# avlmaps/AVLMaps

Measured on AMD Instinct MI355X. Metric: voxel_query_similarities_per_sec, higher is better.
Workload: dtype f32

## Files before the change

avlmaps_amd/csrc/avl_sim.hip:

```cpp
#include <cfloat>
#include <algorithm>
#include <climits>
#include <cstdlib>
#include <vector>

#include "avl_common.h"

namespace avl {

using half8 = __attribute__((ext_vector_type(8))) _Float16;
using half2 = __attribute__((ext_vector_type(2))) _Float16;
using f32x16 = __attribute__((ext_vector_type(16))) float;
using f32x4 = __attribute__((ext_vector_type(4))) float;

constexpr int kExactQB = 8;

template <bool VEC4>
__global__ __launch_bounds__(256) void sim_exact_kernel(const float* __restrict__ feat, int64_t N, int D, int64_t ld,
                                                        const float* __restrict__ q, int Q, int64_t ldq, int q0,
                                                        float* __restrict__ scores, int32_t* __restrict__ argmax,
                                                        float* __restrict__ best, int first_chunk) {
    extern __shared__ __attribute__((aligned(16))) float qs[];
    const int Dp = (D + 3) & ~3;
    const int qn = min(kExactQB, Q - q0);
    for (int i = threadIdx.x; i < kExactQB * Dp; i += blockDim.x) {
        int j = i / Dp, d = i - j * Dp;
        qs[i] = (j < qn && d < D) ? q[(int64_t)(q0 + j) * ldq + d] : 0.f;
    }
    __syncthreads();

    const int lane = threadIdx.x & 63;
    const int64_t wave = (int64_t)blockIdx.x * (blockDim.x >> 6) + (threadIdx.x >> 6);
    const int64_t nwaves = (int64_t)gridDim.x * (blockDim.x >> 6);
    constexpr int R = 4;

    for (int64_t row0 = wave * R; row0 < N; row0 += nwaves * R) {
// ... 148 lines not shown
    const float x[8] = {v0.x, v0.y, v0.z, v0.w, v1.x, v1.y, v1.z, v1.w};
    float m1 = -1.0f;
    asm("" : "+v"(m1));
#pragma unroll
    for (int p = 0; p < 4; ++p) {
        half2 h = __builtin_bit_cast(half2, __builtin_amdgcn_cvt_pkrtz(x[2 * p], x[2 * p + 1]));
        float r0 = __builtin_fmaf((float)h[0], m1, x[2 * p]);
        float r1 = __builtin_fmaf((float)h[1], m1, x[2 * p + 1]);
        half2 l = __builtin_bit_cast(half2, __builtin_amdgcn_cvt_pkrtz(r0, r1));
        hi[2 * p] = h[0];
        hi[2 * p + 1] = h[1];
        lo[2 * p] = l[0];
        lo[2 * p + 1] = l[1];
    }
#endif
}

constexpr float kGuardLo = 0x1p-7f, kGuardHi = 0x1p15f;

__device__ __forceinline__ void guard_max8(float& m, const f32x4 v0, const f32x4 v1) {
#ifndef AVL_GUARD_BUILTIN
    asm("v_max3_f32 %0, |%1|, |%2|, %0" : "+v"(m) : "v"(v0.x), "v"(v0.y));
    asm("v_max3_f32 %0, |%1|, |%2|, %0" : "+v"(m) : "v"(v0.z), "v"(v0.w));
    asm("v_max3_f32 %0, |%1|, |%2|, %0" : "+v"(m) : "v"(v1.x), "v"(v1.y));
    asm("v_max3_f32 %0, |%1|, |%2|, %0" : "+v"(m) : "v"(v1.z), "v"(v1.w));
#else
    m = __builtin_fmaxf(__builtin_fmaxf(m, __builtin_fabsf(v0.x)), __builtin_fabsf(v0.y));
    m = __builtin_fmaxf(__builtin_fmaxf(m, __builtin_fabsf(v0.z)), __builtin_fabsf(v0.w));
    m = __builtin_fmaxf(__builtin_fmaxf(m, __builtin_fabsf(v1.x)), __builtin_fabsf(v1.y));
    m = __builtin_fmaxf(__builtin_fmaxf(m, __builtin_fabsf(v1.z)), __builtin_fabsf(v1.w));
#endif
}

template <int QT, int NA, bool XR = false>
__device__ __forceinline__ void split_epilogue(const f32x16 (&acc)[QT][NA], const float* isc, int q_base, int rows, int Q,
                                               float* __restrict__ scores, int32_t* __restrict__ argmax,
                                               float* __restrict__ best, int64_t row, int64_t N, int kg, int first_chunk,
                                               float rscale = 1.f, uint32_t* __restrict__ flags = nullptr, float rmax = 1.f,
                                               const int32_t* qml = nullptr, f32x4 xacc = f32x4{0.f, 0.f, 0.f, 0.f}) {
    int lim = (XR ? 32 * QT : rows) - 4 * kg;
    asm volatile("" : "+v"(lim));
    float bv = -INFINITY;
    int bl = INT_MAX;
#pragma unroll
    for (int t = 0; t < QT; ++t) {
#pragma unroll
        for (int g = 0; g < 4; ++g) {
            const int c0 = t * 32 + 8 * g;
            const int ql = c0 + 4 * kg;
            const int qg = q_base + ql;
            const f32x4 is4 = *reinterpret_cast<const f32x4*>(isc + ql);
            f32x4 v;
            f32x4 r = {acc[t][0][4 * g + 0], acc[t][0][4 * g + 1], acc[t][0][4 * g + 2], acc[t][0][4 * g + 3]};
#pragma unroll
            for (int a = 1; a < NA; ++a) {
                r.x += acc[t][a][4 * g + 0]; r.y += acc[t][a][4 * g + 1]; r.z += acc[t][a][4 * g + 2]; r.w += acc[t][a][4 * g + 3];
            }
            v.x = r.x * is4.x * rscale;
            v.y = r.y * is4.y * rscale;
            v.z = r.z * is4.z * rscale;
            v.w = r.w * is4.w * rscale;
            if (scores && row < N) {
                float* sp = scores + row * (int64_t)Q + qg;
                if (qml) {
                    float* sr = scores + row * (int64_t)Q;
                    const int4 qm4 = *reinterpret_cast<const int4*>(qml + ql);
                    if (c0 + 0 < lim) sr[qm4.x] = v.x;
                    if (c0 + 1 < lim) sr[qm4.y] = v.y;
                    if (c0 + 2 < lim) sr[qm4.z] = v.z;
                    if (c0 + 3 < lim) sr[qm4.w] = v.w;
                } else if (c0 + 3 < lim && (Q & 3) == 0) {
                    *reinterpret_cast<f32x4*>(sp) = v;
                } else {
                    if (c0 + 0 < lim) sp[0] = v.x;
                    if (c0 + 1 < lim) sp[1] = v.y;
                    if (c0 + 2 < lim) sp[2] = v.z;
                    if (c0 + 3 < lim) sp[3] = v.w;
                }
            }
            if (c0 + 0 < lim && v.x > bv) { bv = v.x; bl = c0 + 0; }
            if (c0 + 1 < lim && v.y > bv) { bv = v.y; bl = c0 + 1; }
            if (c0 + 2 < lim && v.z > bv) { bv = v.z; bl = c0 + 2; }
            if (c0 + 3 < lim && v.w > bv) { bv = v.w; bl = c0 + 3; }
        }
    }
    int bi = bl == INT_MAX ? INT_MAX : q_base + 4 * kg + bl;
    float xv[4] = {0.f, 0.f, 0.f, 0.f};
    if constexpr (XR) {
        const f32x4 xis = *reinterpret_cast<const f32x4*>(isc + 32 * QT);
#pragma unroll
        for (int r = 0; r < 4; ++r) xv[r] = (xacc[r] + __shfl_xor(xacc[r], 32, 64)) * xis[r] * rscale;
        if (scores && row < N && kg == 0) {
            float* sr = scores + row * (int64_t)Q;
#pragma unroll
            for (int r = 0; r < 4; ++r)
                if (32 * QT + r < rows) sr[qml ? qml[32 * QT + r] : q_base + 32 * QT + r] = xv[r];
        }
    }
    if (argmax || best || flags) {
        if (qml && bi != INT_MAX) bi = qml[bi - q_base];
        const float ov = __shfl_xor(bv, 32, 64);
        const int oi = __shfl_xor(bi, 32, 64);
        if (ov > bv || (ov == bv && oi < bi)) {
            bv = ov;
            bi = oi;
        }
        if constexpr (XR) {
#pragma unroll
            for (int r = 0; r < 4; ++r)
                if (32 * QT + r < rows && xv[r] > bv) {
                    bv = xv[r];
                    bi = qml ? qml[32 * QT + r] : q_base + 32 * QT + r;
                }
        }
        if (flags) {
            const float m = fmaxf(rmax, __shfl_xor(rmax, 32, 64));
            const bool bad = row < N && (!(m == 0.f || (m >= kGuardLo && m < kGuardHi)) || bi == INT_MAX);
            const unsigned long long mask = __ballot(bad);
            const int64_t row0 = __shfl(row, 0, 64);
            if ((threadIdx.x & 63) == 0 && row0 < N) {
                const uint32_t w = (uint32_t)(mask | (mask >> 32));
                flags[row0 >> 5] = first_chunk ? w : (flags[row0 >> 5] | w);
            }
        }
        if ((argmax || best) && kg == 0 && row < N) {
            if (bi == INT_MAX) bi = qml ? qml[0] : q_base;
            if (!first_chunk) {
                const float pv = best[row];
                const int pi = argmax ? argmax[row] : -1;
                if (pv > bv || (pv == bv && pi < bi)) {
                    bv = pv;
// ... 164 lines not shown
#else
    (void)hi2;
    const unsigned pat = __builtin_amdgcn_perm(0x54545454u, w, PAIR == 0 ? 0x04010400u : 0x04030402u);
    return __builtin_bit_cast(half2, pat) + half2{(_Float16)-72.0f, (_Float16)-72.0f};
#endif
}

__device__ __forceinline__ void compact_operands(const f32x4& hi, const f32x4& lo, int second, half8& bh, half8& bl) {
    bh = __builtin_bit_cast(half8, hi);
    using u32x4 = __attribute__((ext_vector_type(4))) unsigned;
    const u32x4 hw = __builtin_bit_cast(u32x4, hi);
    const u32x4 lw = __builtin_bit_cast(u32x4, lo);
    const unsigned w0 = lw[second * 2], w1 = lw[second * 2 + 1];
    const half2 l0 = residual_pair<0>(w0, hw[0]), l1 = residual_pair<1>(w0, hw[1]);
    const half2 l2 = residual_pair<0>(w1, hw[2]), l3 = residual_pair<1>(w1, hw[3]);
    bl = half8{l0[0], l0[1], l1[0], l1[1], l2[0], l2[1], l3[0], l3[1]};
}

template <bool PRE, bool P24>
__device__ __forceinline__ void map_operands(const f32x4 (&b)[8], int m, half8& bh, half8& bl, float& rmax) {
    if constexpr (P24) {
        compact_operands(b[m], b[4 + (m >> 1)], m & 1, bh, bl);
    } else if constexpr (PRE) {
        bh = __builtin_bit_cast(half8, b[2 * m]);
        bl = __builtin_bit_cast(half8, b[2 * m + 1]);
    } else {
#ifndef AVL_ABL_NOGUARD
        guard_max8(rmax, b[2 * m], b[2 * m + 1]);
#endif
        split8(b[2 * m], b[2 * m + 1], bh, bl);
    }
}

template <int QT, int NSTEPS, bool PRE, bool FQ, bool QM = false, bool P24 = false, bool XR = false>
__global__ __launch_bounds__(kSplitThreads) void sim_split_f16_kernel(
    const float* __restrict__ feat, int64_t N, int D, int64_t ld, const _Float16* __restrict__ img,
    const float* __restrict__ inv_scale, const float* __restrict__ q_raw, int64_t ldq, int Qtot, int KC, int nkc, int q_base,
    int rows, int Q, float* __restrict__ scores, int32_t* __restrict__ argmax, float* __restrict__ best, int first_chunk,
    const float* __restrict__ row_scale, uint32_t* __restrict__ flags, const int32_t* __restrict__ qmap, int col0) {
    extern __shared__ __attribute__((aligned(16))) char smem[];
    constexpr int NA = QT == 1 ? 3 : (QT == 2 ? 2 : 1);
    constexpr int X1 = NA > 1 ? 1 : 0, X2 = NA > 2 ? 2 : X1;
    const int lane = threadIdx.x & 63, wave = threadIdx.x >> 6;
    const int j = lane & 31, kg = lane >> 5;
    const int row_b = (KC + kRowPadHalves) * 2;
    static_assert(!XR || FQ, "the extra-row path builds its query image in the kernel");
    constexpr int TQ = (QT + (XR ? 1 : 0)) * 32;
    const int zrow = (FQ && rows < (XR ? 32 * QT + 4 : 32 * QT)) ? 1 : 0;
    const int img_b = (rows + zrow) * row_b;
    float* isc = reinterpret_cast<float*>(smem + 2 * img_b);
    int32_t* qml = reinterpret_cast<int32_t*>(isc + TQ);
    if constexpr (QM) {
        if (threadIdx.x < TQ) qml[threadIdx.x] = threadIdx.x < rows ? qmap[q_base + threadIdx.x] : INT_MAX;
    }
    if constexpr (!FQ) {
        if (threadIdx.x < TQ) isc[threadIdx.x] = threadIdx.x < rows ? inv_scale[q_base + threadIdx.x] : 0.f;
    } else {
        if (threadIdx.x >= rows && threadIdx.x < TQ) isc[threadIdx.x] = 0.f;
        constexpr int RB = 4, NW = kSplitThreads / 64;
        for (int r0 = wave; r0 < rows; r0 += NW * RB) {
            float v[RB][8];
#pragma unroll
            for (int b = 0; b < RB; ++b) {
                const int r = r0 + NW * b;
                const float* qr = q_raw + (int64_t)(q_base + (r < rows ? r : rows - 1)) * ldq;
#pragma unroll
                for (int t = 0; t < 8; ++t) v[b][t] = (lane + 64 * t < D) ? qr[lane + 64 * t] : 0.f;
            }
#pragma unroll
            for (int b = 0; b < RB; ++b) {
                const int r = r0 + NW * b;
                if (r < rows) {
                    float m = 0.f;
#pragma unroll
                    for (int t = 0; t < 8; ++t) m = fmaxf(m, fabsf(v[b][t]));
                    for (int off = 32; off > 0; off >>= 1) m = fmaxf(m, __shfl_xor(m, off, 64));
                    int S = 0;
                    if (m > 0.f && isfinite(m)) S = 9 - ilogbf(m);
                    S = max(-60, min(60, S));
// ... 182 lines not shown
                    compute_with([&](int m, half8& bh, half8& bl) {
                        compact_operands(hb[st & 1][m], lb[(st >> 1) & 1][2 * (st & 1) + (m >> 1)], m & 1, bh, bl);
                    }, st);
                }
            } else if constexpr (NSTEPS > 0) {
                constexpr int kRing = RingDepth<PRE, XR, QM>::value;
                f32x4 ring[kRing][8];
#pragma unroll
                for (int r = 0; r + 1 < kRing; ++r)
                    if (r < NSTEPS) load(ring[r], r);
#pragma unroll
                for (int s = 0; s < NSTEPS; ++s) {
                    if (s + kRing - 1 < NSTEPS) load(ring[(s + kRing - 1) % kRing], s + kRing - 1);
                    __builtin_amdgcn_sched_barrier(0);
                    compute(ring[s % kRing], s);
                }
            } else {
                load(buf0, 0);
                for (int s = 0; s < nsteps; s += 2) {
                    if (s + 1 < nsteps) load(buf1, s + 1);
                    compute(buf0, s);
                    if (s + 1 < nsteps) {
                        if (s + 2 < nsteps) load(buf0, s + 2);
                        compute(buf1, s + 1);
                    }
                }
            }
        }

        float rscale = 1.f;
        if constexpr (PRE) {
            if (row_scale) rscale = row_scale[rowc];
        }
        split_epilogue<QT, NA, XR>(acc, isc, q_base, rows, Q, scores, argmax, best, row, N, kg, first_chunk, rscale, PRE ? nullptr : flags, rmax,
                                   QM ? qml : nullptr, xacc0 + xacc1);
    }
}

template <int QT, int T, int NS, bool PRE, bool QM = false, bool P24 = false>
__global__ __launch_bounds__(kSplitThreads) void sim_kswap_f16_kernel(
    const float* __restrict__ feat, int64_t N, int D, int64_t ld, const _Float16* __restrict__ img,
    const float* __restrict__ inv_scale, int Qtot, int KC, int q_base, int rows, int Q, float* __restrict__ scores,
    int32_t* __restrict__ argmax, float* __restrict__ best, int first_chunk, const float* __restrict__ row_scale,
    uint32_t* __restrict__ flags, const int32_t* __restrict__ qmap, int col0) {
    extern __shared__ __attribute__((aligned(16))) char smem[];
    const int lane = threadIdx.x & 63, wave = threadIdx.x >> 6;
    const int j = lane & 31, kg = lane >> 5;
    const int row_b = (KC + kRowPadHalves) * 2;
    const int zrow = rows < 32 * QT ? 1 : 0;
    const int img_b = (rows + zrow) * row_b;
    float* isc = reinterpret_cast<float*>(smem + 2 * img_b);
    int32_t* qml = reinterpret_cast<int32_t*>(isc + QT * 32);
    if constexpr (QM) {
        if (threadIdx.x < QT * 32) qml[threadIdx.x] = threadIdx.x < rows ? qmap[q_base + threadIdx.x] : INT_MAX;
    }
    if (threadIdx.x < QT * 32) isc[threadIdx.x] = threadIdx.x < rows ? inv_scale[q_base + threadIdx.x] : 0.f;
    auto fill_lds = [&](int kc) {
        using gptr = const __attribute__((address_space(1))) void*;
        using lptr = __attribute__((address_space(3))) void*;
        const char* hi = reinterpret_cast<const char*>(img) + ((int64_t)(kc * 2) * Qtot + q_base) * row_b;
        const char* lo = hi + (int64_t)Qtot * row_b;
        const int nb = rows * row_b;
        for (int c = wave * 1024; c < nb; c += (kSplitThreads / 64) * 1024) {
            if (c + lane * 16 < nb) {
                __builtin_amdgcn_global_load_lds((gptr)(hi + c + lane * 16), (lptr)(smem + c), 16, 0, 0);
                __builtin_amdgcn_global_load_lds((gptr)(lo + c + lane * 16), (lptr)(smem + img_b + c), 16, 0, 0);
            }
        }
// ... 693 lines not shown
                si[threadIdx.x] = oi;
            }
        }
        __syncthreads();
    }
    if (threadIdx.x == 0) {
        pv[blockIdx.x] = sv[0];
        pi[blockIdx.x] = si[0];
    }
}

struct SplitChunk {
    int q_base, rows, QT;
};

struct SplitPlan {
    int Qtot, KC, nkc, nchunks, max_rows;
    bool stream;
    bool kswap;
    int SPC;
    SplitChunk chunks[64];
    size_t hdr_bytes, ws_bytes;
    size_t lds_bytes(const SplitChunk& c) const {
        if (stream) return (size_t)2 * (c.rows + 1) * (2 * KC + kRowPadHalves) * 2 + (size_t)c.QT * 32 * 2 * sizeof(float);
        return (size_t)4 * (c.rows + 1) * (KC + kRowPadHalves) + (size_t)c.QT * 32 * 2 * sizeof(float);
    }
};

#ifndef AVL_SIM_EXTRA_ROWS
#define AVL_SIM_EXTRA_ROWS 1
#endif
constexpr bool kSimExtraRows = AVL_SIM_EXTRA_ROWS != 0;
constexpr size_t kLdsBudget = 163840 - 512;

static bool stream_fits(int rows, int KS) {
    const size_t buf = (size_t)rows * (2 * KS + kRowPadHalves) * 2;
    const size_t zero_row = (size_t)(2 * KS + kRowPadHalves) * 2;
    return 2 * (buf + zero_row) + 256 * sizeof(float) <= kLdsBudget && buf <= (size_t)kStreamFill * kSplitThreads * 16;
}

static bool make_split_plan(int D, int Q, SplitPlan& p, bool allow_stream = true) {
    if (D % 64 != 0 || D <= 0 || Q <= 0) return false;
    p.stream = false;
    p.kswap = false;
    p.SPC = 0;
    p.Qtot = (Q + 31) / 32 * 32;
    const int kc0 = D < 512 ? D : 512;
    int r3 = (int)((kLdsBudget - 192 * sizeof(float)) / (4 * (size_t)(kc0 + kRowPadHalves))) - 1;
    if (r3 > 96) r3 = 96;
    const int npass = (Q + r3 - 1) / r3;
    if (npass > 64) return false;
    const int per = (Q + npass - 1) / npass;
    p.nchunks = 0;
    p.max_rows = 0;
    for (int base = 0; base < Q; base += per) {
        const int take = Q - base < per ? Q - base : per;
        p.chunks[p.nchunks++] = SplitChunk{base, take, (take + 31) / 32};
        if (take > p.max_rows) p.max_rows = take;
    }
    int kcmax = (int)((kLdsBudget - 192 * sizeof(float)) / (4 * (size_t)(p.max_rows + 1))) - kRowPadHalves;
    kcmax = (kcmax / 64) * 64;
    if (kcmax < 64) return false;
    p.nkc = (D + kcmax - 1) / kcmax;
    const int kc = (D + p.nkc - 1) / p.nkc;
    p.KC = ((kc + 63) / 64) * 64;
    p.nkc = (D + p.KC - 1) / p.KC;
    p.hdr_bytes = (((size_t)p.Qtot * sizeof(float)) + kHdrAlign - 1) / kHdrAlign * kHdrAlign;
    p.ws_bytes = p.hdr_bytes + (size_t)p.nkc * 2 * p.Qtot * (p.KC + kRowPadHalves) * sizeof(_Float16);
    static const bool kswap_on = [] { const char* e = std::getenv("AVL_SIM_KSWAP"); return !(e && e[0] == '0'); }();
    p.kswap = kswap_on && allow_stream && p.nkc == 2 && p.nchunks == 1 && p.max_rows <= 64;
    if (p.kswap) return true;
    if (allow_stream && D % 128 == 0) {
        const int npass_s = (Q + 127) / 128;
        const int per_s = (Q + npass_s - 1) / npass_s;
        if (npass_s <= 64 && (p.nkc > 1 || npass_s < p.nchunks)) {
            const int spc = (D % 256 == 0 && stream_fits(per_s, 256)) ? 4 : 2;
            if (stream_fits(per_s, 64 * spc)) {
                p.stream = true;
                p.SPC = spc;
                p.KC = 64 * spc;
                p.nkc = D / p.KC;
                p.nchunks = 0;
                p.max_rows = 0;
                for (int base = 0; base < Q; base += per_s) {
                    const int take = Q - base < per_s ? Q - base : per_s;
                    p.chunks[p.nchunks++] = SplitChunk{base, take, (take + 31) / 32};
                    if (take > p.max_rows) p.max_rows = take;
                }
                p.ws_bytes = p.hdr_bytes + (size_t)p.nkc * p.Qtot * (2 * p.KC + kRowPadHalves) * sizeof(_Float16);
            }
        }
    }
    return true;
}

static int ensure_dynamic_lds(const void* kern, size_t bytes) {
    struct Entry { const void* k; size_t bytes; int dev; };
    static thread_local Entry table[64];
    static thread_local int used = 0;
    int dev = 0;
    (void)hipGetDevice(&dev);
    for (int i = 0; i < used; ++i)
        if (table[i].k == kern && table[i].dev == dev) {
            if (table[i].bytes >= bytes) return AVL_OK;
            AVL_HIP_CHECK(hipFuncSetAttribute(kern, hipFuncAttributeMaxDynamicSharedMemorySize, (int)bytes));
            table[i].bytes = bytes;
            return AVL_OK;
        }
    AVL_HIP_CHECK(hipFuncSetAttribute(kern, hipFuncAttributeMaxDynamicSharedMemorySize, (int)bytes));
    if (used < 64) table[used++] = Entry{kern, bytes, dev};
    return AVL_OK;
}

static int run_exact(const float* d_feat, int64_t N, int D, int64_t ld, const float* d_q, int Q, int64_t ldq,
                     float* d_scores, int32_t* d_argmax, float* d_best, hipStream_t st) {
    const int Dp = (D + 3) & ~3;
    const size_t lds = (size_t)kExactQB * Dp * sizeof(float);
    AVL_REQUIRE(lds <= 160 * 1024, "avl_sim_scores: D=%d too large for the exact path", D);
    const bool vec4 = (D % 4 == 0) && (ld % 4 == 0) && ((reinterpret_cast<uintptr_t>(d_feat) & 15) == 0);
    const int waves_per_block = 4;
    int64_t blocks = (N + waves_per_block * 4 - 1) / (waves_per_block * 4);
    const int64_t maxb = (int64_t)num_cus() * 8;
    if (blocks > maxb) blocks = maxb;
    if (blocks < 1) blocks = 1;
    auto kern = vec4 ? sim_exact_kernel<true> : sim_exact_kernel<false>;
    if (lds > 64 * 1024) {
        int rc = ensure_dynamic_lds(reinterpret_cast<const void*>(kern), lds);
        if (rc != AVL_OK) return rc;
    }
    for (int q0 = 0, first = 1; q0 < Q; q0 += kExactQB, first = 0) {
        hipLaunchKernelGGL(kern, dim3((unsigned)blocks), dim3(256), lds, st, d_feat, N, D, ld, d_q, Q, ldq, q0, d_scores,
                           d_argmax, d_best, first);
    }
    AVL_HIP_CHECK(hipGetLastError());
    return AVL_OK;
}

template <int SPC, bool PRE, bool QM, bool P24 = false>
static const void* pick_stream_kernel(int QT, bool tile_block) {
    if (tile_block && QT == 2) return reinterpret_cast<const void*>(sim_stream_tb_f16_kernel<2, SPC, PRE, QM, P24>);
    switch (QT) {
        case 1: return reinterpret_cast<const void*>(sim_stream_f16_kernel<1, SPC, PRE, QM, P24>);
        case 2: return reinterpret_cast<const void*>(sim_stream_f16_kernel<2, SPC, PRE, QM, P24>);
        case 3: return reinterpret_cast<const void*>(sim_stream_f16_kernel<3, SPC, PRE, QM, P24>);
        default: return reinterpret_cast<const void*>(sim_stream_f16_kernel<4, SPC, PRE, QM, P24>);
    }
}

template <bool PRE, bool QM, bool P24>
static const void* pick_stream_kernel_spc(int SPC, int QT, bool tile_block) {
    return SPC == 4 ? pick_stream_kernel<4, PRE, QM, P24>(QT, tile_block) : pick_stream_kernel<2, PRE, QM, P24>(QT, tile_block);
}

#ifndef AVL_KSWAP_T
#define AVL_KSWAP_T 3
#endif
template <int NS, bool PRE, bool QM, bool P24>
static const void* pick_kswap_kernel_ns(int QT) {
    if (QT == 2) return reinterpret_cast<const void*>(sim_kswap_f16_kernel<2, AVL_KSWAP_T, NS, PRE, QM, P24>);
    return reinterpret_cast<const void*>(sim_kswap_f16_kernel<1, 2 * AVL_KSWAP_T, 0, PRE, QM, P24>);
}
template <bool PRE, bool QM, bool P24>
static const void* pick_kswap_kernel(int QT, int ns) {
    return ns == 8 ? pick_kswap_kernel_ns<8, PRE, QM, P24>(QT) : (ns == 6 ? pick_kswap_kernel_ns<6, PRE, QM, P24>(QT) : pick_kswap_kernel_ns<0, PRE, QM, P24>(QT));
}

static bool split_plan_is_fused(const SplitPlan& p, int D) { return !p.stream && p.nkc == 1 && D <= 512; }

template <int QT, bool QM>
static const void* pick_split24_kernel(bool s8, bool fq) {
    if (fq) return s8 ? reinterpret_cast<const void*>(sim_split_f16_kernel<QT, 8, true, true, QM, true>)
                      : reinterpret_cast<const void*>(sim_split_f16_kernel<QT, 0, true, true, QM, true>);
    return reinterpret_cast<const void*>(sim_split_f16_kernel<QT, 0, true, false, QM, true>);
}

template <int QT>
static const void* pick_split_xr_kernel(bool prepared, bool p24) {
    if (p24) return reinterpret_cast<const void*>(sim_split_f16_kernel<QT, 8, true, true, false, true, true>);
    if (prepared) return reinterpret_cast<const void*>(sim_split_f16_kernel<QT, 8, true, true, false, false, true>);
    return reinterpret_cast<const void*>(sim_split_f16_kernel<QT, 8, false, true, false, false, true>);
}

template <int QT, bool PRE, bool QM>
static const void* pick_split_kernel(bool s8, bool fq) {
    if (fq) return s8 ? reinterpret_cast<const void*>(sim_split_f16_kernel<QT, 8, PRE, true, QM>)
                      : reinterpret_cast<const void*>(sim_split_f16_kernel<QT, 0, PRE, true, QM>);
    return reinterpret_cast<const void*>(sim_split_f16_kernel<QT, 0, PRE, false, QM>);
}

static int run_fixup(const float* d_feat, int64_t N, int D, int64_t ld, const float* d_q, int Q, int64_t ldq, const uint32_t* d_flags,
                     float* d_scores, int32_t* d_argmax, float* d_best, hipStream_t st) {
    const int64_t nwords = (N + 31) >> 5;
    int64_t blocks = (nwords + 255) / 256;
    const int64_t maxb = (int64_t)num_cus() * 8;
    if (blocks > maxb) blocks = maxb;
    if (blocks < 1) blocks = 1;
    hipLaunchKernelGGL(sim_fixup_rows_kernel, dim3((unsigned)blocks), dim3(256), 0, st, d_feat, N, D, ld, d_q, Q, ldq, d_flags, d_scores,
                       d_argmax, d_best);
    AVL_HIP_CHECK(hipGetLastError());
    return AVL_OK;
}

template <bool PRE>
static int run_split(const float* d_feat, int64_t N, int D, int64_t ld, const float* d_q, int Qg, int64_t ldq, int Qs,
                     float* d_scores, int32_t* d_argmax, float* d_best, const SplitPlan& p, void* d_ws, const float* d_row_scale,
                     uint32_t* d_flags, const int32_t* d_qmap, bool first_launch, hipStream_t st, bool p24 = false, int col0 = 0) {
    float* inv_scale = reinterpret_cast<float*>(d_ws);
    _Float16* img = reinterpret_cast<_Float16*>(reinterpret_cast<char*>(d_ws) + p.hdr_bytes);
    const bool fq = split_plan_is_fused(p, D);
    if (!fq)
        hipLaunchKernelGGL(sim_prep_queries_kernel, dim3(p.Qtot), dim3(256), 0, st, d_q, Qg, D, ldq, inv_scale, img, p.Qtot, p.KC,
                           p.nkc, p.stream ? 1 : 0);
    const int64_t ntiles = (N + kTileRows - 1) / kTileRows;
    int64_t blocks = ntiles < num_cus() ? ntiles : num_cus();
    if (blocks < 1) blocks = 1;
    if (p.stream) {
        for (int ci = 0; ci < p.nchunks; ++ci) {
            const SplitChunk& c = p.chunks[ci];
            const bool tb = ((ld * (p24 ? 3 : 4)) % 4096) != 0;
            const void* kern = nullptr;
            if constexpr (PRE) {
                if (p24) kern = d_qmap ? pick_stream_kernel_spc<true, true, true>(p.SPC, c.QT, tb) : pick_stream_kernel_spc<true, false, true>(p.SPC, c.QT, tb);
// ... 8 lines not shown
            void* args[] = {&d_feat, &N, &D, &ld, &img_c, &isc_c, &Qtot, &nch, &q_base, &rows, &Qs, &d_scores, &d_argmax, &d_best, &first,
                            &d_row_scale, &d_flags, &d_qmap, &col0};
            AVL_HIP_CHECK(hipLaunchKernel(kern, dim3((unsigned)blocks), dim3(kSplitThreads), args, lds, st));
        }
        AVL_HIP_CHECK(hipGetLastError());
        return AVL_OK;
    }
    if (p.kswap) {
        const SplitChunk& c = p.chunks[0];
        const int s8 = (p24 && col0 % 128 != 0) ? 0 : ((p.KC == 512 && D == 1024) ? 8 : ((p.KC == 384 && D == 768) ? 6 : 0));
        const void* kern = nullptr;
        if constexpr (PRE) {
            if (p24) kern = d_qmap ? pick_kswap_kernel<true, true, true>(c.QT, s8) : pick_kswap_kernel<true, false, true>(c.QT, s8);
        }
        if (!kern) kern = d_qmap ? pick_kswap_kernel<PRE, true, false>(c.QT, s8) : pick_kswap_kernel<PRE, false, false>(c.QT, s8);
        const size_t lds = p.lds_bytes(c);
        int rc = ensure_dynamic_lds(kern, lds);
        if (rc != AVL_OK) return rc;
        const _Float16* img_c = img;
        const float* isc_c = inv_scale;
        int Qtot = p.Qtot, KC = p.KC, q_base = c.q_base, rows = c.rows, first = first_launch ? 1 : 0;
        void* args[] = {&d_feat, &N, &D, &ld, &img_c, &isc_c, &Qtot, &KC, &q_base, &rows, &Qs, &d_scores, &d_argmax, &d_best, &first,
                        &d_row_scale, &d_flags, &d_qmap, &col0};
        AVL_HIP_CHECK(hipLaunchKernel(kern, dim3((unsigned)blocks), dim3(kSplitThreads), args, lds, st));
        AVL_HIP_CHECK(hipGetLastError());
        return AVL_OK;
    }
    for (int ci = 0; ci < p.nchunks; ++ci) {
        const SplitChunk& c = p.chunks[ci];
        const bool s8 = (p.nkc == 1 && D == 512) && (!p24 || col0 % 128 == 0);
        const int xr = c.rows % 32;
        const bool use_xr = kSimExtraRows && s8 && fq && !d_qmap && xr >= 1 && xr <= 4 && c.rows > 32 && c.rows / 32 <= 2 &&
                            (PRE || c.rows / 32 == 2);
        const void* kern = use_xr ? (c.rows / 32 == 2 ? pick_split_xr_kernel<2>(PRE, p24) : pick_split_xr_kernel<1>(PRE, p24))
                           : (p24 && d_qmap) ? (c.QT == 3 ? pick_split24_kernel<3, true>(s8, fq) : (c.QT == 2 ? pick_split24_kernel<2, true>(s8, fq) : pick_split24_kernel<1, true>(s8, fq)))
                           : p24  ? (c.QT == 3 ? pick_split24_kernel<3, false>(s8, fq) : (c.QT == 2 ? pick_split24_kernel<2, false>(s8, fq) : pick_split24_kernel<1, false>(s8, fq)))
                           : d_qmap ? (c.QT == 3 ? pick_split_kernel<3, PRE, true>(s8, fq)
                                               : (c.QT == 2 ? pick_split_kernel<2, PRE, true>(s8, fq) : pick_split_kernel<1, PRE, true>(s8, fq)))
                                  : (c.QT == 3 ? pick_split_kernel<3, PRE, false>(s8, fq)
                                               : (c.QT == 2 ? pick_split_kernel<2, PRE, false>(s8, fq) : pick_split_kernel<1, PRE, false>(s8, fq)));
        const size_t lds = p.lds_bytes(c);
        int rc = ensure_dynamic_lds(kern, lds);
        if (rc != AVL_OK) return rc;
        const _Float16* img_c = img;
        const float* isc_c = inv_scale;
        int Qtot = p.Qtot, KC = p.KC, nkc = p.nkc, q_base = c.q_base, rows = c.rows, first = (ci == 0 && first_launch) ? 1 : 0;
        void* args[] = {&d_feat, &N, &D, &ld, &img_c, &isc_c, &d_q, &ldq, &Qtot, &KC, &nkc, &q_base, &rows, &Qs,
                        &d_scores, &d_argmax, &d_best, &first, &d_row_scale, &d_flags, &d_qmap, &col0};
        AVL_HIP_CHECK(hipLaunchKernel(kern, dim3((unsigned)blocks), dim3(kSplitThreads), args, lds, st));
    }
    AVL_HIP_CHECK(hipGetLastError());
    return AVL_OK;
}

static int run_mfma_f32(const float* d_feat, int64_t N, int D, int64_t ld, const float* d_q, int Q, int64_t ldq,
                        float* d_scores, int32_t* d_argmax, float* d_best, const SplitPlan& p, void* d_ws, hipStream_t st) {
    float* img = reinterpret_cast<float*>(d_ws);
    hipLaunchKernelGGL(sim_prep_queries_f32_kernel, dim3(p.Qtot), dim3(256), 0, st, d_q, Q, D, ldq, img, p.Qtot, p.KC, p.nkc);
    const int64_t ntiles = (N + kTileRows - 1) / kTileRows;
    int64_t blocks = ntiles < num_cus() ? ntiles : num_cus();
    if (blocks < 1) blocks = 1;
    for (int ci = 0; ci < p.nchunks; ++ci) {
        const SplitChunk& c = p.chunks[ci];
        auto kern = c.QT == 3 ? sim_mfma_f32_kernel<3> : (c.QT == 2 ? sim_mfma_f32_kernel<2> : sim_mfma_f32_kernel<1>);
        const size_t lds = (size_t)c.rows * (p.KC + kRowPadF32) * sizeof(float);
        int rc = ensure_dynamic_lds(reinterpret_cast<const void*>(kern), lds);
        if (rc != AVL_OK) return rc;
        hipLaunchKernelGGL(kern, dim3((unsigned)blocks), dim3(kSplitThreads), lds, st, d_feat, N, D, ld, img, p.Qtot, p.KC, p.nkc, c.q_base,
                           c.rows, Q, d_scores, d_argmax, d_best, ci == 0 ? 1 : 0);
    }
    AVL_HIP_CHECK(hipGetLastError());
    return AVL_OK;
}

}

using namespace avl;

extern "C" {

static size_t align_up(size_t b, size_t a) { return (b + a - 1) / a * a; }
// ... 332 lines not shown
```

Measured before the change: 177.6 billion.

## Stage split-kernel score stores through a per-wave LDS slab for coalesced writes

```diff
diff --git a/avlmaps_amd/csrc/avl_sim.hip b/avlmaps_amd/csrc/avl_sim.hip
--- a/avlmaps_amd/csrc/avl_sim.hip
+++ b/avlmaps_amd/csrc/avl_sim.hip
@@ -2,6 +2,7 @@
 #include <algorithm>
 #include <climits>
 #include <cstdlib>
+#include <cstring>
 #include <vector>
 
 #include "avl_common.h"
@@ -216,6 +217,102 @@
 #endif
 }
 
+template <int QT, int NA>
+__device__ __forceinline__ f32x4 epilogue_scores4(const f32x16 (&acc)[QT][NA], int t, int g, const float* is4p, float rscale) {
+    const f32x4 is4 = *reinterpret_cast<const f32x4*>(is4p);
+    f32x4 r = {acc[t][0][4 * g + 0], acc[t][0][4 * g + 1], acc[t][0][4 * g + 2], acc[t][0][4 * g + 3]};
+#pragma unroll
+    for (int a = 1; a < NA; ++a) {
+        r.x += acc[t][a][4 * g + 0]; r.y += acc[t][a][4 * g + 1]; r.z += acc[t][a][4 * g + 2]; r.w += acc[t][a][4 * g + 3];
+    }
+    f32x4 v;
+    v.x = r.x * is4.x * rscale;
+    v.y = r.y * is4.y * rscale;
+    v.z = r.z * is4.z * rscale;
+    v.w = r.w * is4.w * rscale;
+    return v;
+}
+
+__device__ __forceinline__ void epilogue_extra4(float (&xv)[4], const f32x4 xacc, const float* xisp, float rscale) {
+    const f32x4 xis = *reinterpret_cast<const f32x4*>(xisp);
+#pragma unroll
+    for (int r = 0; r < 4; ++r) xv[r] = (xacc[r] + __shfl_xor(xacc[r], 32, 64)) * xis[r] * rscale;
+}
+
+template <int QT, int NA, bool XR>
+__device__ __forceinline__ void slab_store_scores(const f32x16 (&acc)[QT][NA], const float* isc, int Q, float* __restrict__ scores,
+                                                  int64_t row, int64_t N, int lane, float rscale, f32x4 xacc, float* slab, int R) {
+    const int j = lane & 31, kg = lane >> 5;
+    const int64_t row0 = row - j;
+    const int valid = N - row0 < 32 ? (int)(N - row0) : 32;
+    const bool vec = (Q & 3) == 0;
+    const int nC = Q >> 2;
+    const int kmask = (vec && (nC & 1) == 0) ? 7 : 0;
+    const int ks = kmask ? max(3, __builtin_ctz(nC)) : 3;
+    int lim = (XR ? 32 * QT : Q) - 4 * kg;
+    asm volatile("" : "+v"(lim));
+    float xv[4] = {0.f, 0.f, 0.f, 0.f};
+    if constexpr (XR) epilogue_extra4(xv, xacc, isc + 32 * QT, rscale);
+    auto slot = [&](int lin) {
+        const int o = lin >> 2;
+        return ((o ^ ((o >> ks) & kmask)) << 2) | (lin & 3);
+    };
+    f32x4 v[QT][4];
+#pragma unroll
+    for (int t = 0; t < QT; ++t)
+#pragma unroll
+        for (int g = 0; g < 4; ++g) v[t][g] = epilogue_scores4<QT, NA>(acc, t, g, isc + t * 32 + 8 * g + 4 * kg, rscale);
+    for (int r0 = 0; r0 < valid; r0 += R) {
+        const int rl = j - r0;
+        if (rl >= 0 && rl < R) {
+            const int lin0 = rl * Q + 4 * kg;
+            if (vec) {
+#pragma unroll
+                for (int t = 0; t < QT; ++t)
+#pragma unroll
+                    for (int g = 0; g < 4; ++g)
+                        if (t * 32 + 8 * g < lim) *reinterpret_cast<f32x4*>(slab + slot(lin0 + t * 32 + 8 * g)) = v[t][g];
+            } else {
+#pragma unroll
+                for (int t = 0; t < QT; ++t)
+#pragma unroll
+                    for (int g = 0; g < 4; ++g) {
+                        const int c0 = t * 32 + 8 * g;
+                        if (c0 + 0 < lim) slab[lin0 + c0 + 0] = v[t][g].x;
+                        if (c0 + 1 < lim) slab[lin0 + c0 + 1] = v[t][g].y;
+                        if (c0 + 2 < lim) slab[lin0 + c0 + 2] = v[t][g].z;
+                        if (c0 + 3 < lim) slab[lin0 + c0 + 3] = v[t][g].w;
+                    }
+            }
+            if constexpr (XR) {
+                if (kg == 0) {
+#pragma unroll
+                    for (int r = 0; r < 4; ++r)
+                        if (32 * QT + r < Q) slab[slot(rl * Q + 32 * QT + r)] = xv[r];
+                }
+            }
+        }
+        __builtin_amdgcn_fence(__ATOMIC_RELEASE, "wavefront");
+        __builtin_amdgcn_wave_barrier();
+        __builtin_amdgcn_fence(__ATOMIC_ACQUIRE, "wavefront");
+        const int ndw = (valid - r0 < R ? valid - r0 : R) * Q;
+        float* gp = scores + (row0 + r0) * (int64_t)Q;
+        for (int o = lane; 4 * o < ndw; o += 64) {
+            const f32x4 w = *reinterpret_cast<const f32x4*>(slab + ((o ^ ((o >> ks) & kmask)) << 2));
+            if (4 * o + 3 < ndw) {
+                *reinterpret_cast<f32x4*>(gp + 4 * o) = w;
+            } else {
+                gp[4 * o] = w.x;
+                if (4 * o + 1 < ndw) gp[4 * o + 1] = w.y;
+                if (4 * o + 2 < ndw) gp[4 * o + 2] = w.z;
+            }
+        }
+        __builtin_amdgcn_fence(__ATOMIC_RELEASE, "wavefront");
+        __builtin_amdgcn_wave_barrier();
+        __builtin_amdgcn_fence(__ATOMIC_ACQUIRE, "wavefront");
+    }
+}
+
 template <int QT, int NA, bool XR = false>
 __device__ __forceinline__ void split_epilogue(const f32x16 (&acc)[QT][NA], const float* isc, int q_base, int rows, int Q,
                                                float* __restrict__ scores, int32_t* __restrict__ argmax,
@@ -233,17 +330,7 @@
             const int c0 = t * 32 + 8 * g;
             const int ql = c0 + 4 * kg;
             const int qg = q_base + ql;
-            const f32x4 is4 = *reinterpret_cast<const f32x4*>(isc + ql);
-            f32x4 v;
-            f32x4 r = {acc[t][0][4 * g + 0], acc[t][0][4 * g + 1], acc[t][0][4 * g + 2], acc[t][0][4 * g + 3]};
-#pragma unroll
-            for (int a = 1; a < NA; ++a) {
-                r.x += acc[t][a][4 * g + 0]; r.y += acc[t][a][4 * g + 1]; r.z += acc[t][a][4 * g + 2]; r.w += acc[t][a][4 * g + 3];
-            }
-            v.x = r.x * is4.x * rscale;
-            v.y = r.y * is4.y * rscale;
-            v.z = r.z * is4.z * rscale;
-            v.w = r.w * is4.w * rscale;
+            const f32x4 v = epilogue_scores4<QT, NA>(acc, t, g, isc + ql, rscale);
             if (scores && row < N) {
                 float* sp = scores + row * (int64_t)Q + qg;
                 if (qml) {
@@ -271,9 +358,7 @@
     int bi = bl == INT_MAX ? INT_MAX : q_base + 4 * kg + bl;
     float xv[4] = {0.f, 0.f, 0.f, 0.f};
     if constexpr (XR) {
-        const f32x4 xis = *reinterpret_cast<const f32x4*>(isc + 32 * QT);
-#pragma unroll
-        for (int r = 0; r < 4; ++r) xv[r] = (xacc[r] + __shfl_xor(xacc[r], 32, 64)) * xis[r] * rscale;
+        epilogue_extra4(xv, xacc, isc + 32 * QT, rscale);
         if (scores && row < N && kg == 0) {
             float* sr = scores + row * (int64_t)Q;
 #pragma unroll
@@ -511,12 +596,13 @@
     }
 }
 
-template <int QT, int NSTEPS, bool PRE, bool FQ, bool QM = false, bool P24 = false, bool XR = false>
+template <int QT, int NSTEPS, bool PRE, bool FQ, bool QM = false, bool P24 = false, bool XR = false, bool SLAB = false>
 __global__ __launch_bounds__(kSplitThreads) void sim_split_f16_kernel(
     const float* __restrict__ feat, int64_t N, int D, int64_t ld, const _Float16* __restrict__ img,
     const float* __restrict__ inv_scale, const float* __restrict__ q_raw, int64_t ldq, int Qtot, int KC, int nkc, int q_base,
     int rows, int Q, float* __restrict__ scores, int32_t* __restrict__ argmax, float* __restrict__ best, int first_chunk,
-    const float* __restrict__ row_scale, uint32_t* __restrict__ flags, const int32_t* __restrict__ qmap, int col0) {
+    const float* __restrict__ row_scale, uint32_t* __restrict__ flags, const int32_t* __restrict__ qmap, int col0, int slab_off,
+    int slab_rows) {
     extern __shared__ __attribute__((aligned(16))) char smem[];
     constexpr int NA = QT == 1 ? 3 : (QT == 2 ? 2 : 1);
     constexpr int X1 = NA > 1 ? 1 : 0, X2 = NA > 2 ? 2 : X1;
@@ -524,6 +610,7 @@
     const int j = lane & 31, kg = lane >> 5;
     const int row_b = (KC + kRowPadHalves) * 2;
     static_assert(!XR || FQ, "the extra-row path builds its query image in the kernel");
+    static_assert(!SLAB || (FQ && !QM), "the score slab serves one dense query chunk and needs a tile loop without barriers");
     constexpr int TQ = (QT + (XR ? 1 : 0)) * 32;
     const int zrow = (FQ && rows < (XR ? 32 * QT + 4 : 32 * QT)) ? 1 : 0;
     const int img_b = (rows + zrow) * row_b;
@@ -772,8 +859,15 @@
         if constexpr (PRE) {
             if (row_scale) rscale = row_scale[rowc];
         }
-        split_epilogue<QT, NA, XR>(acc, isc, q_base, rows, Q, scores, argmax, best, row, N, kg, first_chunk, rscale, PRE ? nullptr : flags, rmax,
-                                   QM ? qml : nullptr, xacc0 + xacc1);
+        if constexpr (SLAB) {
+            const int wave_u = __builtin_amdgcn_readfirstlane(wave);
+            float* slab = reinterpret_cast<float*>(smem + slab_off) + wave_u * (((slab_rows * Q + 31) >> 5) << 5);
+            int lane_o = lane;
+            asm volatile("" : "+v"(lane_o));
+            slab_store_scores<QT, NA, XR>(acc, isc, Q, scores, row, N, lane_o, rscale, xacc0 + xacc1, slab, slab_rows);
+        }
+        split_epilogue<QT, NA, XR>(acc, isc, q_base, rows, Q, SLAB ? nullptr : scores, argmax, best, row, N, kg, first_chunk, rscale,
+                                   PRE ? nullptr : flags, rmax, QM ? qml : nullptr, xacc0 + xacc1);
     }
 }
 
@@ -1689,6 +1783,39 @@
     return reinterpret_cast<const void*>(sim_split_f16_kernel<QT, 0, PRE, false, QM>);
 }
 
+template <int NS, bool XR>
+static const void* pick_split_slab_kernel_ns(int full, bool prepared, bool p24) {
+    if constexpr (!XR) {
+        if (full == 3)
+            return p24 ? reinterpret_cast<const void*>(sim_split_f16_kernel<3, NS, true, true, false, true, false, true>)
+                       : prepared ? reinterpret_cast<const void*>(sim_split_f16_kernel<3, NS, true, true, false, false, false, true>)
+                                  : reinterpret_cast<const void*>(sim_split_f16_kernel<3, NS, false, true, false, false, false, true>);
+    }
+    if (full == 2)
+        return p24 ? reinterpret_cast<const void*>(sim_split_f16_kernel<2, NS, true, true, false, true, XR, true>)
+                   : prepared ? reinterpret_cast<const void*>(sim_split_f16_kernel<2, NS, true, true, false, false, XR, true>)
+                              : reinterpret_cast<const void*>(sim_split_f16_kernel<2, NS, false, true, false, false, XR, true>);
+    return p24 ? reinterpret_cast<const void*>(sim_split_f16_kernel<1, NS, true, true, false, true, XR, true>)
+               : prepared ? reinterpret_cast<const void*>(sim_split_f16_kernel<1, NS, true, true, false, false, XR, true>)
+                          : reinterpret_cast<const void*>(sim_split_f16_kernel<1, NS, false, true, false, false, XR, true>);
+}
+static const void* pick_split_slab_kernel(int full, bool prepared, bool p24, bool s8, bool xr) {
+    if (xr) return pick_split_slab_kernel_ns<8, true>(full, prepared, p24);
+    return s8 ? pick_split_slab_kernel_ns<8, false>(full, prepared, p24) : pick_split_slab_kernel_ns<0, false>(full, prepared, p24);
+}
+
+static int score_slab_rows(size_t used, int Q, size_t& off) {
+    static const bool lanes = [] { const char* e = std::getenv("AVL_SIM_SCORE_STORE"); return e && std::strcmp(e, "lanes") == 0; }();
+    if (lanes) return 0;
+    off = (used + 127) / 128 * 128;
+    for (int r = 32; r >= 2; r >>= 1) {
+        if (((int64_t)r * Q) % 4 != 0) break;
+        const size_t per_wave = ((size_t)r * Q * 4 + 127) / 128 * 128;
+        if (off + (kSplitThreads / 64) * per_wave <= kLdsBudget) return r;
+    }
+    return 0;
+}
+
 static int run_fixup(const float* d_feat, int64_t N, int D, int64_t ld, const float* d_q, int Q, int64_t ldq, const uint32_t* d_flags,
                      float* d_scores, int32_t* d_argmax, float* d_best, hipStream_t st) {
     const int64_t nwords = (N + 31) >> 5;
@@ -1770,14 +1897,21 @@
                                                : (c.QT == 2 ? pick_split_kernel<2, PRE, true>(s8, fq) : pick_split_kernel<1, PRE, true>(s8, fq)))
                                   : (c.QT == 3 ? pick_split_kernel<3, PRE, false>(s8, fq)
                                                : (c.QT == 2 ? pick_split_kernel<2, PRE, false>(s8, fq) : pick_split_kernel<1, PRE, false>(s8, fq)));
-        const size_t lds = p.lds_bytes(c);
+        size_t lds = p.lds_bytes(c);
+        size_t slab_off_b = 0;
+        int slab_rows = (d_scores && fq && !d_qmap && p.nchunks == 1) ? score_slab_rows(lds, Qs, slab_off_b) : 0;
+        if (slab_rows) {
+            kern = pick_split_slab_kernel(use_xr ? c.rows / 32 : c.QT, PRE, p24, s8, use_xr);
+            lds = slab_off_b + (kSplitThreads / 64) * (((size_t)slab_rows * Qs * 4 + 127) / 128 * 128);
+        }
+        int slab_off = (int)slab_off_b;
         int rc = ensure_dynamic_lds(kern, lds);
         if (rc != AVL_OK) return rc;
         const _Float16* img_c = img;
         const float* isc_c = inv_scale;
         int Qtot = p.Qtot, KC = p.KC, nkc = p.nkc, q_base = c.q_base, rows = c.rows, first = (ci == 0 && first_launch) ? 1 : 0;
         void* args[] = {&d_feat, &N, &D, &ld, &img_c, &isc_c, &d_q, &ldq, &Qtot, &KC, &nkc, &q_base, &rows, &Qs,
-                        &d_scores, &d_argmax, &d_best, &first, &d_row_scale, &d_flags, &d_qmap, &col0};
+                        &d_scores, &d_argmax, &d_best, &first, &d_row_scale, &d_flags, &d_qmap, &col0, &slab_off, &slab_rows};
         AVL_HIP_CHECK(hipLaunchKernel(kern, dim3((unsigned)blocks), dim3(kSplitThreads), args, lds, st));
     }
     AVL_HIP_CHECK(hipGetLastError());
```

New measurement: 178.0 billion, median of 6. Within noise of the previous version (+0.2%).

## Stage score tiles through LDS for coalesced row-contiguous global stores

Applied to the files above, without the earlier changes.

```diff
diff --git a/avlmaps_amd/csrc/avl_sim.hip b/avlmaps_amd/csrc/avl_sim.hip
--- a/avlmaps_amd/csrc/avl_sim.hip
+++ b/avlmaps_amd/csrc/avl_sim.hip
@@ -216,16 +216,92 @@
 #endif
 }
 
-template <int QT, int NA, bool XR = false>
+__device__ __forceinline__ void wave_lds_exchange() {
+    __builtin_amdgcn_fence(__ATOMIC_RELEASE, "wavefront");
+    __builtin_amdgcn_wave_barrier();
+    __builtin_amdgcn_fence(__ATOMIC_ACQUIRE, "wavefront");
+}
+
+template <int QT, bool XR>
+__device__ __forceinline__ void store_scores_staged(const f32x4 (&sv)[QT][4], const float (&xv)[4], int lim, int rows, int Q,
+                                                    float* __restrict__ scores, int64_t row, int64_t N, char* stage0) {
+    int tid = threadIdx.x;
+    asm volatile("" : "+v"(tid));
+    const int lane = tid & 63, j = lane & 31, kg = lane >> 5;
+    char* stage = stage0 + (tid >> 6) * (32 * Q);
+    const int64_t r0 = row - j;
+    const int64_t row0 = ((int64_t)__builtin_amdgcn_readfirstlane((int)(r0 >> 32)) << 32) | (uint32_t)__builtin_amdgcn_readfirstlane((int)r0);
+    const int nvalid = (int)(N - row0 < 32 ? N - row0 : 32);
+    const int pass_b = 32 * Q;
+    char* gblk = reinterpret_cast<char*>(scores + row0 * (int64_t)Q);
+#ifdef AVL_ABL_LINEAR_STORE
+    (void)stage; (void)xv; (void)lim; (void)rows; (void)pass_b; (void)kg;
+#pragma unroll
+    for (int i = 0; i < 4 * QT; ++i)
+        if (16 * lane + 1024 * i + 16 <= nvalid * 4 * Q) *reinterpret_cast<f32x4*>(gblk + 16 * lane + 1024 * i) = sv[i >> 2][i & 3];
+    return;
+#endif
+    float* wr = reinterpret_cast<float*>(stage) + (j & 7) * Q;
+#pragma unroll 1
+    for (int p = 0; p < 4; ++p) {
+        const int lim_b = (nvalid - 8 * p < 8 ? nvalid - 8 * p : 8) * 4 * Q;
+        if (lim_b <= 0) break;
+        if ((j >> 3) == p) {
+#pragma unroll
+            for (int t = 0; t < QT; ++t) {
+#pragma unroll
+                for (int g = 0; g < 4; ++g) {
+                    const int c0 = t * 32 + 8 * g;
+                    const bool full = XR || t + 1 < QT;
+                    float* w = wr + c0 + 4 * kg;
+                    if (full || c0 + 0 < lim) w[0] = sv[t][g].x;
+                    if (full || c0 + 1 < lim) w[1] = sv[t][g].y;
+                    if (full || c0 + 2 < lim) w[2] = sv[t][g].z;
+                    if (full || c0 + 3 < lim) w[3] = sv[t][g].w;
+                }
+            }
+            if constexpr (XR) {
+                if (kg == 0) {
+#pragma unroll
+                    for (int r = 0; r < 4; ++r)
+                        if (32 * QT + r < rows) wr[32 * QT + r] = xv[r];
+                }
+            }
+        }
+        wave_lds_exchange();
+#pragma unroll
+        for (int i = 0; i < QT + (XR ? 1 : 0); ++i) {
+            const int o = 16 * lane + 1024 * i;
+            if (o < lim_b) {
+                const f32x4 d = *reinterpret_cast<const f32x4*>(stage + o);
+                char* gp = gblk + (int64_t)p * pass_b + o;
+                if (o + 16 <= lim_b) {
+                    *reinterpret_cast<f32x4*>(gp) = d;
+                } else {
+                    float* gf = reinterpret_cast<float*>(gp);
+                    gf[0] = d.x;
+                    if (o + 8 <= lim_b) gf[1] = d.y;
+                    if (o + 12 <= lim_b) gf[2] = d.z;
+                }
+            }
+        }
+        wave_lds_exchange();
+    }
+}
+
+template <int QT, int NA, bool XR = false, bool SC = false>
 __device__ __forceinline__ void split_epilogue(const f32x16 (&acc)[QT][NA], const float* isc, int q_base, int rows, int Q,
                                                float* __restrict__ scores, int32_t* __restrict__ argmax,
                                                float* __restrict__ best, int64_t row, int64_t N, int kg, int first_chunk,
                                                float rscale = 1.f, uint32_t* __restrict__ flags = nullptr, float rmax = 1.f,
-                                               const int32_t* qml = nullptr, f32x4 xacc = f32x4{0.f, 0.f, 0.f, 0.f}) {
+                                               const int32_t* qml = nullptr, f32x4 xacc = f32x4{0.f, 0.f, 0.f, 0.f},
+                                               char* stage = nullptr) {
     int lim = (XR ? 32 * QT : rows) - 4 * kg;
     asm volatile("" : "+v"(lim));
     float bv = -INFINITY;
     int bl = INT_MAX;
+    f32x4 sv[SC ? QT : 1][4];
+    (void)sv;
 #pragma unroll
     for (int t = 0; t < QT; ++t) {
 #pragma unroll
@@ -244,7 +320,9 @@
             v.y = r.y * is4.y * rscale;
             v.z = r.z * is4.z * rscale;
             v.w = r.w * is4.w * rscale;
-            if (scores && row < N) {
+            if constexpr (SC) {
+                sv[t][g] = v;
+            } else if (scores && row < N) {
                 float* sp = scores + row * (int64_t)Q + qg;
                 if (qml) {
                     float* sr = scores + row * (int64_t)Q;
@@ -274,13 +352,14 @@
         const f32x4 xis = *reinterpret_cast<const f32x4*>(isc + 32 * QT);
 #pragma unroll
         for (int r = 0; r < 4; ++r) xv[r] = (xacc[r] + __shfl_xor(xacc[r], 32, 64)) * xis[r] * rscale;
-        if (scores && row < N && kg == 0) {
+        if (!SC && scores && row < N && kg == 0) {
             float* sr = scores + row * (int64_t)Q;
 #pragma unroll
             for (int r = 0; r < 4; ++r)
                 if (32 * QT + r < rows) sr[qml ? qml[32 * QT + r] : q_base + 32 * QT + r] = xv[r];
         }
     }
+    if constexpr (SC) store_scores_staged<QT, XR>(sv, xv, lim, rows, Q, scores, row, N, stage);
     if (argmax || best || flags) {
         if (qml && bi != INT_MAX) bi = qml[bi - q_base];
         const float ov = __shfl_xor(bv, 32, 64);
@@ -511,7 +590,7 @@
     }
 }
 
-template <int QT, int NSTEPS, bool PRE, bool FQ, bool QM = false, bool P24 = false, bool XR = false>
+template <int QT, int NSTEPS, bool PRE, bool FQ, bool QM = false, bool P24 = false, bool XR = false, bool SC = false>
 __global__ __launch_bounds__(kSplitThreads) void sim_split_f16_kernel(
     const float* __restrict__ feat, int64_t N, int D, int64_t ld, const _Float16* __restrict__ img,
     const float* __restrict__ inv_scale, const float* __restrict__ q_raw, int64_t ldq, int Qtot, int KC, int nkc, int q_base,
@@ -524,6 +603,7 @@
     const int j = lane & 31, kg = lane >> 5;
     const int row_b = (KC + kRowPadHalves) * 2;
     static_assert(!XR || FQ, "the extra-row path builds its query image in the kernel");
+    static_assert(!SC || (FQ && !QM), "staged scores: a dense launch over whole rows, no barrier in the tile loop");
     constexpr int TQ = (QT + (XR ? 1 : 0)) * 32;
     const int zrow = (FQ && rows < (XR ? 32 * QT + 4 : 32 * QT)) ? 1 : 0;
     const int img_b = (rows + zrow) * row_b;
@@ -772,8 +852,9 @@
         if constexpr (PRE) {
             if (row_scale) rscale = row_scale[rowc];
         }
-        split_epilogue<QT, NA, XR>(acc, isc, q_base, rows, Q, scores, argmax, best, row, N, kg, first_chunk, rscale, PRE ? nullptr : flags, rmax,
-                                   QM ? qml : nullptr, xacc0 + xacc1);
+        split_epilogue<QT, NA, XR, SC>(acc, isc, q_base, rows, Q, scores, argmax, best, row, N, kg, first_chunk, rscale, PRE ? nullptr : flags, rmax,
+                                       QM ? qml : nullptr, xacc0 + xacc1,
+                                       SC ? smem + 2 * img_b + 2 * TQ * (int)sizeof(float) : nullptr);
     }
 }
 
@@ -1533,6 +1614,10 @@
 #endif
 constexpr bool kSimExtraRows = AVL_SIM_EXTRA_ROWS != 0;
 constexpr size_t kLdsBudget = 163840 - 512;
+#ifndef AVL_SIM_STAGED_SCORES
+#define AVL_SIM_STAGED_SCORES 1
+#endif
+constexpr bool kSimStagedScores = AVL_SIM_STAGED_SCORES != 0;
 
 static bool stream_fits(int rows, int KS) {
     const size_t buf = (size_t)rows * (2 * KS + kRowPadHalves) * 2;
@@ -1597,7 +1682,7 @@
 
 static int ensure_dynamic_lds(const void* kern, size_t bytes) {
     struct Entry { const void* k; size_t bytes; int dev; };
-    static thread_local Entry table[64];
+    static thread_local Entry table[192];
     static thread_local int used = 0;
     int dev = 0;
     (void)hipGetDevice(&dev);
@@ -1609,7 +1694,7 @@
             return AVL_OK;
         }
     AVL_HIP_CHECK(hipFuncSetAttribute(kern, hipFuncAttributeMaxDynamicSharedMemorySize, (int)bytes));
-    if (used < 64) table[used++] = Entry{kern, bytes, dev};
+    if (used < 192) table[used++] = Entry{kern, bytes, dev};
     return AVL_OK;
 }
 
@@ -1669,21 +1754,34 @@
 static bool split_plan_is_fused(const SplitPlan& p, int D) { return !p.stream && p.nkc == 1 && D <= 512; }
 
 template <int QT, bool QM>
-static const void* pick_split24_kernel(bool s8, bool fq) {
+static const void* pick_split24_kernel(bool s8, bool fq, bool sc = false) {
+    if constexpr (!QM && QT > 1) {
+        if (sc) return s8 ? reinterpret_cast<const void*>(sim_split_f16_kernel<QT, 8, true, true, false, true, false, true>)
+                          : reinterpret_cast<const void*>(sim_split_f16_kernel<QT, 0, true, true, false, true, false, true>);
+    }
     if (fq) return s8 ? reinterpret_cast<const void*>(sim_split_f16_kernel<QT, 8, true, true, QM, true>)
                       : reinterpret_cast<const void*>(sim_split_f16_kernel<QT, 0, true, true, QM, true>);
     return reinterpret_cast<const void*>(sim_split_f16_kernel<QT, 0, true, false, QM, true>);
 }
 
 template <int QT>
-static const void* pick_split_xr_kernel(bool prepared, bool p24) {
+static const void* pick_split_xr_kernel(bool prepared, bool p24, bool sc) {
+    if (sc) {
+        if (p24) return reinterpret_cast<const void*>(sim_split_f16_kernel<QT, 8, true, true, false, true, true, true>);
+        if (prepared) return reinterpret_cast<const void*>(sim_split_f16_kernel<QT, 8, true, true, false, false, true, true>);
+        return reinterpret_cast<const void*>(sim_split_f16_kernel<QT, 8, false, true, false, false, true, true>);
+    }
     if (p24) return reinterpret_cast<const void*>(sim_split_f16_kernel<QT, 8, true, true, false, true, true>);
     if (prepared) return reinterpret_cast<const void*>(sim_split_f16_kernel<QT, 8, true, true, false, false, true>);
     return reinterpret_cast<const void*>(sim_split_f16_kernel<QT, 8, false, true, false, false, true>);
 }
 
 template <int QT, bool PRE, bool QM>
-static const void* pick_split_kernel(bool s8, bool fq) {
+static const void* pick_split_kernel(bool s8, bool fq, bool sc = false) {
+    if constexpr (!QM && QT > 1) {
+        if (sc) return s8 ? reinterpret_cast<const void*>(sim_split_f16_kernel<QT, 8, PRE, true, false, false, false, true>)
+                          : reinterpret_cast<const void*>(sim_split_f16_kernel<QT, 0, PRE, true, false, false, false, true>);
+    }
     if (fq) return s8 ? reinterpret_cast<const void*>(sim_split_f16_kernel<QT, 8, PRE, true, QM>)
                       : reinterpret_cast<const void*>(sim_split_f16_kernel<QT, 0, PRE, true, QM>);
     return reinterpret_cast<const void*>(sim_split_f16_kernel<QT, 0, PRE, false, QM>);
@@ -1763,14 +1861,17 @@
         const int xr = c.rows % 32;
         const bool use_xr = kSimExtraRows && s8 && fq && !d_qmap && xr >= 1 && xr <= 4 && c.rows > 32 && c.rows / 32 <= 2 &&
                             (PRE || c.rows / 32 == 2);
-        const void* kern = use_xr ? (c.rows / 32 == 2 ? pick_split_xr_kernel<2>(PRE, p24) : pick_split_xr_kernel<1>(PRE, p24))
+        const size_t stage_b = (size_t)(kSplitThreads / 64) * 32 * Qs;
+        const bool sc = kSimStagedScores && fq && d_scores && !d_qmap && p.nchunks == 1 && c.rows == Qs && Qs > 32 && (Qs & 3) != 0 &&
+                        (reinterpret_cast<uintptr_t>(d_scores) & 15) == 0 && p.lds_bytes(c) + stage_b <= kLdsBudget;
+        const void* kern = use_xr ? (c.rows / 32 == 2 ? pick_split_xr_kernel<2>(PRE, p24, sc) : pick_split_xr_kernel<1>(PRE, p24, sc))
                            : (p24 && d_qmap) ? (c.QT == 3 ? pick_split24_kernel<3, true>(s8, fq) : (c.QT == 2 ? pick_split24_kernel<2, true>(s8, fq) : pick_split24_kernel<1, true>(s8, fq)))
-                           : p24  ? (c.QT == 3 ? pick_split24_kernel<3, false>(s8, fq) : (c.QT == 2 ? pick_split24_kernel<2, false>(s8, fq) : pick_split24_kernel<1, false>(s8, fq)))
+                           : p24  ? (c.QT == 3 ? pick_split24_kernel<3, false>(s8, fq, sc) : (c.QT == 2 ? pick_split24_kernel<2, false>(s8, fq, sc) : pick_split24_kernel<1, false>(s8, fq, sc)))
                            : d_qmap ? (c.QT == 3 ? pick_split_kernel<3, PRE, true>(s8, fq)
                                                : (c.QT == 2 ? pick_split_kernel<2, PRE, true>(s8, fq) : pick_split_kernel<1, PRE, true>(s8, fq)))
-                                  : (c.QT == 3 ? pick_split_kernel<3, PRE, false>(s8, fq)
-                                               : (c.QT == 2 ? pick_split_kernel<2, PRE, false>(s8, fq) : pick_split_kernel<1, PRE, false>(s8, fq)));
-        const size_t lds = p.lds_bytes(c);
+                                  : (c.QT == 3 ? pick_split_kernel<3, PRE, false>(s8, fq, sc)
+                                               : (c.QT == 2 ? pick_split_kernel<2, PRE, false>(s8, fq, sc) : pick_split_kernel<1, PRE, false>(s8, fq, sc)));
+        const size_t lds = p.lds_bytes(c) + (sc ? stage_b : 0);
         int rc = ensure_dynamic_lds(kern, lds);
         if (rc != AVL_OK) return rc;
         const _Float16* img_c = img;
```

Result: slower. 181.3 billion before, 178.3 billion after (-1.6%).
